# epsilla-cloud/vectordb

Measured on AMD Instinct MI355X. Metric: QPS @ recall@10>=0.999, 10Mx768 L2, higher is better.
Workload: dtype f32 (exact fp32 distances; the batched scan runs an int8 MFMA pass (int32 accumulation) over an 8-bit mirror of the rows as a lower-bound filter, survivors re-ranked in fp32)

## Files before the change

### vectordb_amd/csrc/flat_kernels.hip

```cpp
#include "kernels.hpp"
#include "stream8_kernel.hpp"

namespace eps {

template <int NQ, int KPL>
__device__ __forceinline__ void offer(WaveTopK<KPL> (&list)[NQ], u64 (&thr)[NQ], int q, u64 key, bool valid,
                                      const FilterSpec& f, int k, bool unique) {
  u64 m = __ballot(valid && key < thr[q]);
  while (m) {
    const int l = __ffsll((long long)m) - 1;
    m &= m - 1;
    const u64 x = shfl64(key, l);
    if (x < thr[q] && row_visible(f, key_id(x), key_dist(x))) {
      if (unique) list[q].insert_unique(x); else list[q].insert(x);
      const u64 kth = list[q].entry(k - 1);
      thr[q] = kth < thr[q] ? kth : thr[q];
    }
  }
}

template <int NQ, int KPL, bool VEC4, int U>
__global__ __launch_bounds__(256) void flat_scan_kernel(FlatScanArgs a) {
  extern __shared__ __attribute__((aligned(16))) float smem[];
  const int dim = a.dim;
// ... 445 lines not shown
    if (lost_s) atomicAdd(a.overflow, 1u);
    if (a.fuse & 1) {
      if (cnt_raw > (u32)S8R_CAP || cnt_raw > (u32)a.cap) atomicAdd(a.overflow, 1u);
      atomicAdd(a.total, (unsigned long long)cnt);
    }
    a.cand_count[q] = 0;
    if (a.pub) {
      __threadfence();
      if (atomicAdd(a.pub_ticket, 1u) == gridDim.x - 1) {
        const u32 ov = atomicAdd(a.overflow, 0u);
        const unsigned long long tot = atomicAdd(a.total, 0ull);
        a.pub[0] = ov;
        a.pub[2] = (u32)tot;
        a.pub[3] = (u32)(tot >> 32);
        __threadfence_system();
        if (a.s8_reset) {
          *a.overflow = 0u;
          *a.total = 0ull;
          *a.pub_ticket = 0u;
        }
      }
    }
  }
}

void launch_rerank(const RerankArgs& a, hipStream_t s) {
  if (a.nq <= 0) return;
  if (a.s8_G && a.s8_fast && pick_kpl(a.k) == 1 && a.s8_waves <= S8_MAX_WAVES && !a.T_next && !a.gsync) {
    const bool v4 = (a.dim % 4 == 0) && ((reinterpret_cast<uintptr_t>(a.rows) & 15) == 0);
    const size_t sm = (size_t)((a.dim + 3) & ~3) * sizeof(float) + (size_t)S8R_CAP * sizeof(u64);
    if (v4) hipLaunchKernelGGL((s8_rerank_kernel<true>), dim3((unsigned)a.nq), dim3(1024), sm, s, a);
    else hipLaunchKernelGGL((s8_rerank_kernel<false>), dim3((unsigned)a.nq), dim3(1024), sm, s, a);
    return;
  }
  const bool vec4 = (a.dim % 4 == 0) && ((reinterpret_cast<uintptr_t>(a.rows) & 15) == 0);
  const int kpl = pick_kpl(a.k);
  const int nw = (a.nq <= 64 && kpl <= 4) ? 16 : 4;
  const size_t shm = (size_t)((a.dim + 3) & ~3) * sizeof(float) + (size_t)nw * kpl * 64 * sizeof(u64);
#define EPS_CASE(KPL_)                                                                                               \
  if (kpl == KPL_) {                                                                                                 \
    if (nw == 16) {                                                                                                  \
      if (vec4) hipLaunchKernelGGL((rerank_kernel<KPL_, true, 16>), dim3((unsigned)a.nq), dim3(1024), shm, s, a);    \
      else hipLaunchKernelGGL((rerank_kernel<KPL_, false, 16>), dim3((unsigned)a.nq), dim3(1024), shm, s, a);        \
    } else {                                                                                                         \
      if (vec4) hipLaunchKernelGGL((rerank_kernel<KPL_, true, 4>), dim3((unsigned)a.nq), dim3(256), shm, s, a);      \
      else hipLaunchKernelGGL((rerank_kernel<KPL_, false, 4>), dim3((unsigned)a.nq), dim3(256), shm, s, a);          \
    }                                                                                                                \
    return;                                                                                                          \
  }
  EPS_CASE(1) EPS_CASE(2) EPS_CASE(4) EPS_CASE(8) EPS_CASE(16)
#undef EPS_CASE
}

__global__ void finalize_kernel(const u64* run_keys, int64_t nq, int k, int64_t id_base, int64_t id_stride,
                                int64_t* ids, float* dist, int32_t* counts) {
  const int64_t i = (int64_t)blockIdx.x * blockDim.x + threadIdx.x;
  if (i >= nq * k) return;
  const u64 key = run_keys[i];
  const bool valid = key != KEY_EMPTY;
  ids[i] = valid ? (int64_t)key_id(key) * id_stride + id_base : -1;
  dist[i] = valid ? key_dist(key) : __builtin_inff();
  if (counts && (i % k) == 0) {
    int c = 0;
    for (int e = 0; e < k; ++e) c += run_keys[i + e] != KEY_EMPTY;
    counts[i / k] = c;
  }
}
void launch_finalize(const u64* run_keys, int64_t nq, int k, int64_t id_base, int64_t id_stride, int64_t* ids,
                     float* dist, int32_t* counts, hipStream_t s) {
  const int64_t n = nq * k;
  if (n <= 0) return;
  hipLaunchKernelGGL(finalize_kernel, dim3((unsigned)((n + 255) / 256)), dim3(256), 0, s, run_keys, nq, k, id_base,
                     id_stride, ids, dist, counts);
}

__global__ void fill_u64_kernel(u64* p, int64_t n, u64 v) {
  const int64_t i = (int64_t)blockIdx.x * blockDim.x + threadIdx.x;
  if (i < n) p[i] = v;
}
void launch_fill_u64(u64* p, int64_t n, u64 v, hipStream_t s) {
  if (n <= 0) return;
  hipLaunchKernelGGL(fill_u64_kernel, dim3((unsigned)((n + 255) / 256)), dim3(256), 0, s, p, n, v);
}

__global__ __launch_bounds__(256) void normalize_kernel(float* rows, int64_t n, int dim, int only_if_nonzero) {
  const int64_t r = (int64_t)blockIdx.x * 4 + (threadIdx.x >> 6);
  if (r >= n) return;
  const int lane = lane_id();
  float* p = rows + r * dim;
  float s = 0.f;
  for (int c = lane; c < dim; c += 64) s = fmaf(p[c], p[c], s);
  for (int o = 32; o > 0; o >>= 1) s += __shfl_xor(s, o);
  if (only_if_nonzero && !(s > 1e-10f)) return;
  const float nrm = sqrtf(s);
  for (int c = lane; c < dim; c += 64) p[c] = p[c] / nrm;
}
void launch_normalize(float* rows, int64_t n, int dim, bool only_if_nonzero, hipStream_t s) {
  if (n <= 0) return;
  hipLaunchKernelGGL(normalize_kernel, dim3((unsigned)((n + 3) / 4)), dim3(256), 0, s, rows, n, dim,
                     only_if_nonzero ? 1 : 0);
}

__global__ void merge_shards_kernel(const float* dist, const int64_t* ids, int shards, int64_t nq, int k,
                                    float* out_dist, int64_t* out_ids, int64_t stride_bytes, int32_t* out_counts) {
  const int64_t q = (int64_t)blockIdx.x * blockDim.x + threadIdx.x;
  if (q >= nq) return;
// ... 40 lines not shown
```

### vectordb_amd/csrc/kernels.hpp

```cpp
#pragma once
#include <hip/hip_runtime.h>
#include <stdint.h>

#include "device_common.hpp"

namespace eps {

struct FlatScanArgs {
  const float* rows;
  int64_t row_begin, row_end;
  int dim;
  int metric;
  const float* queries;
  int64_t nq;
  int k;
  FilterSpec f;
  u64* partial;
  int W;
  const u64* thr_in;
  const u64* lo_in;
  int64_t lo_stride;
};
int flat_scan_waves(int64_t nrows, int64_t nq, int dim);
void launch_flat_scan(const FlatScanArgs& a, hipStream_t s);

void launch_merge_lists(const u64* keys, int slots, int k, int64_t nq, u64* run_keys, bool merge_run, hipStream_t s,
                        const u32* counts = nullptr, const FilterSpec* visible = nullptr, u64 id_stride = 0, u32 id_head = 0,
                        u32* seed_cand = nullptr, int seed_cap = 0, u32* seed_cnt = nullptr);

struct RerankArgs {
  const float* rows;
  int dim;
  int metric;
  const float* queries;
  int64_t nq;
  int k;
  FilterSpec f;
  const u32* cand;
  u32* cand_count;
  int cap;
  u64* run_keys;
  int fuse;
  u32* overflow;
  unsigned long long* total;
  void* T_next;
  const float* qstat;
  const float* scal;
  int bits;
  float u, slack;
  u32* gsync;
  int64_t* fin_ids = nullptr;
  float* fin_dist = nullptr;
  int32_t* fin_counts = nullptr;
  int64_t fin_base = 0, fin_stride = 1;
  const int* s8_G = nullptr;
  int s8_slots = 64;
  const u32* s8_counts = nullptr;
  const u64* s8_lists = nullptr;
  int s8_waves = 0;
  u32* s8_cand = nullptr;
  u32* pub = nullptr;
  u32* pub_ticket = nullptr;
  int s8_fast = 0;
  int s8_reset = 0;
};
void launch_rerank(const RerankArgs& a, hipStream_t s);

void launch_finalize(const u64* run_keys, int64_t nq, int k, int64_t id_base, int64_t id_stride, int64_t* ids,
                     float* dist, int32_t* counts, hipStream_t s);

void launch_normalize(float* rows, int64_t n, int dim, bool only_if_nonzero, hipStream_t s);
void launch_merge_shards(const float* dist, const int64_t* ids, int shards, int64_t nq, int k, float* out_dist,
                         int64_t* out_ids, hipStream_t s, int64_t stride_bytes = 0, int32_t* out_counts = nullptr);
void launch_fill_u64(u64* p, int64_t n, u64 v, hipStream_t s);

constexpr int SEL_ROWS = 1024;
constexpr int SEL_THREADS = 256;
constexpr int SEL_SCAN_THREADS = 512;
inline int64_t select_blocks(int64_t n) { return (n + SEL_ROWS - 1) / SEL_ROWS; }
struct SelectArgs {
  FilterSpec f;
  int64_t n;
  int64_t skip, limit;
  int64_t id_base, id_stride;
  u64* bits;
  u32* counts;
  int64_t* offsets;
  int64_t* ids_out;
  int64_t* count_out;
  int64_t* total_out;
};
void launch_select(const SelectArgs& a, hipStream_t s);

}
```

### vectordb_amd/csrc/mfma_filter.hip

```cpp
#include <algorithm>
#include <cmath>
#include <cstdio>
#include <cstring>
#include <numeric>
#include <vector>

#include "mirror.hpp"
#include "mfma_kernels.hpp"

namespace eps {

__global__ __launch_bounds__(256) void query_prep_kernel(const float* q, int64_t nq, int64_t b_pad, int dim, int d_pad,
                                                         _Float16* qh, float* qstat) {
  const int64_t r = (int64_t)blockIdx.x * 4 + (threadIdx.x >> 6);
  if (r >= b_pad) return;
  const int lane = lane_id();
  _Float16* dst = qh + r * d_pad;
  if (r >= nq) {
    for (int c = lane; c < d_pad; c += 64) dst[c] = (_Float16)0.f;
    if (lane == 0) qstat[r * 4 + 0] = qstat[r * 4 + 1] = qstat[r * 4 + 2] = qstat[r * 4 + 3] = 0.f;
    return;
  }
  const float* src = q + r * dim;
  float s2 = 0.f, e2 = 0.f;
// ... 116 lines not shown
    if (i8)
      while (nstages < 8 && (double)k * 5.0 * std::pow((double)n / (double)S0, 1.0 / (double)nstages) > 0.5 * (double)cap) ++nstages;
    const double r = std::max(i8 ? 3.0 : 4.0, std::pow((double)n / (double)S0, 1.0 / (double)nstages));
    const int64_t qt = std::max<int64_t>(1, b_pad / 256);
    const int64_t unit = 256 * std::max<int64_t>(1, 256 / std::gcd<int64_t>(256, qt));
    double f = 1.0;
    for (int st = 1; st < nstages; ++st) {
      f *= r;
      int64_t bnd = (int64_t)((double)S0 * f) / ROWPAD * ROWPAD;
      if (bnd >= 2 * unit) bnd = bnd / unit * unit;
      if (bnd < n && bnd > bounds.back()) bounds.push_back(bnd);
    }
  } else {
    bounds.push_back(std::min(S0, n));
    for (int64_t bnd : {S0 * 32, S0 * 256}) {
      if (bnd < n && bnd > bounds.back()) bounds.push_back(bnd);
    }
  }
  if (bounds.back() < n) bounds.push_back(n);
  return bounds;
}

struct Chain {
  const float* dq; int64_t nq; int k; u64* run_keys;
  bool i8;
  bool approx;
  int64_t n;
  bool fold;
  bool seeded;
  bool prologue;
  bool gsync;
  int version;
  int64_t b_pad, S0;
  int cap;
  int d_pad_h;
  float u8, slack;
  CallCounters c;
  FilterSpec fs;
  std::vector<int64_t> bounds;
  bool prep_does_it_all() const { return i8 && version >= 7; }
  const float* maxima(const HalfMirror& m) const { return i8 ? (fold ? m.scal8f.as<float>() : m.scal8.as<float>()) : m.scal.as<float>(); }
  u32* group_counters(const HalfMirror& m) const { return gsync ? m.gsync.as<u32>() : nullptr; }
};

static int32_t plan_chain(Index& ix, HalfMirror& m, const float* dq, int64_t nq, int k, u64* run_keys, bool approx, int cap_scale, bool i8, int64_t n, Chain* out) {
  Chain& c = *out = Chain{dq, nq, k, run_keys, i8, approx, n};
  c.b_pad = (nq + BN3 - 1) / BN3 * BN3;
  c.cap = std::max(4096, 64 * k) * cap_scale;
  c.d_pad_h = i8 ? m.d_pad8 / 2 : m.d_pad;
  c.u8 = key_unit8(ix.metric_, m.step8);
  c.slack = rerank_slack(ix.dim_);
  const int64_t b_pad = c.b_pad;
  if (!m.qstat.reserve((size_t)b_pad * 16) || !m.T.reserve((size_t)b_pad * 4) || !m.cand.reserve((size_t)nq * c.cap * 8) ||
      !m.cnt.reserve((size_t)(nq + 4) * 4 + 16) || !m.seedc.reserve((size_t)nq * k * 4) || !(i8 ? m.q8.reserve((size_t)b_pad * m.d_pad8) : m.qh.reserve((size_t)b_pad * m.d_pad * 2)))
    return ix.fail(EPS_INFRA_UNEXPECTED_ERROR, "MFMA engine: out of device memory (scratch)");
  c.version = (c.d_pad_h % 128 != 0 || c.d_pad_h < 256) ? 3 : 7;
  if (c.version >= 7 && !m.qf.reserve((size_t)b_pad * c.d_pad_h * 2)) return ix.fail(EPS_INFRA_UNEXPECTED_ERROR, "MFMA engine: out of device memory (scratch)");
  if (!m.gsync.reserve(1024)) return ix.fail(EPS_INFRA_UNEXPECTED_ERROR, "MFMA engine: out of device memory (scratch)");
  c.S0 = seed_rows(k);
  c.seeded = !(tune_int("EPS_MFMA_SEED", 1) == 0) && n > 4 * c.S0;
  c.prologue = c.seeded && c.version >= 7;
  c.gsync = !(tune_int("EPS_MFMA_GROUPSYNC", 1) == 0);
  c.fold = i8 && !approx && m.fold8;
  c.c = call_counters(m.cnt.as<u32>(), nq);
  c.fs = ix.filter_spec();
  c.bounds = plan_stages(n, nq, k, b_pad, c.cap, i8, approx, c.seeded);
  return EPS_OK;
}

static int32_t prepare_queries(Index& ix, HalfMirror& m, const Chain& c) {
  hipStream_t s = ix.stream_;
  if (c.i8) {
    Prep8Extra px;
    if (c.prep_does_it_all()) {
      px.qf = m.qf.as<signed char>();
      if (c.prologue) {
        px.T2 = reinterpret_cast<u64*>(m.T.p);
        px.n2 = c.b_pad / 2;
        px.Tv = 0x7F8000007F800000ull;
        px.cnt = c.c.cnt;
        px.cntv = (u32)c.S0;
        px.gsync = c.group_counters(m);
      }
    }
    const hipError_t er = prep8_queries(m, c.fold, (int)ix.dim_, ix.metric_, c.dq, c.nq, c.b_pad, m.q8.as<signed char>(), m.qstat.as<float>(), px, s);
    if (er != hipSuccess) return ix.hip_fail(er, "memset");
    if (c.fold) ix.stats_.i8_folded = 1;
    ix.stats_.i8_rotated = m.rot8 ? 1 : 0;
  } else {
    hipLaunchKernelGGL(query_prep_kernel, dim3((unsigned)((c.b_pad + 3) / 4)), dim3(256), 0, s, c.dq, c.nq, c.b_pad, (int)ix.dim_,
                       m.d_pad, m.qh.as<_Float16>(), m.qstat.as<float>());
  }
  if (c.version >= 7 && !c.prep_does_it_all())
    hipLaunchKernelGGL(pack_qf_kernel, dim3((unsigned)((c.b_pad / 32) * (c.d_pad_h / 16))), dim3(64), 0, s, m.qh.as<_Float16>(), m.qf.as<_Float16>(), c.b_pad, c.d_pad_h);
  return EPS_OK;
}

static FilterArgs filter_args(const Index& ix, const HalfMirror& m, const Chain& c) {
  const bool i8 = c.i8;
  FilterArgs fa;
  fa.xh = i8 ? reinterpret_cast<const _Float16*>(m.x8.p) : m.xh.as<_Float16>();
  fa.qh = i8 ? reinterpret_cast<const _Float16*>(m.q8.p) : m.qh.as<_Float16>();
  fa.qf = m.qf.as<_Float16>();
  fa.base = i8 ? (c.fold ? m.acc0b.as<float>() : m.acc0.as<float>()) : (ix.metric_ == 0 ? m.xn.as<float>() : m.zeros.as<float>());
  fa.base_s = i8 ? (c.fold ? m.acc0b.as<float>() : m.acc0.as<float>()) : (ix.metric_ == 0 ? m.xn_s.as<float>() : m.zeros_s.as<float>());
  fa.T = m.T.as<float>();
  fa.d_pad = c.d_pad_h;
// ... 59 lines not shown
  hipStream_t s = ix.stream_;
  const bool i8 = c.i8;
  const int64_t S0 = c.S0;
  u32* cnt = c.c.cnt;
  const bool dense = c.version >= 7;
  if (c.prologue && c.prep_does_it_all()) {
  } else if (c.prologue) {
    const int64_t cells = std::max<int64_t>(std::max<int64_t>(c.b_pad / 2, c.nq), 256);
    hipLaunchKernelGGL(seed_prologue_kernel, dim3((unsigned)((cells + 255) / 256)), dim3(256), 0, s, reinterpret_cast<u64*>(m.T.p), c.b_pad / 2, 0x7F8000007F800000ull,
                       cnt, c.nq, (u32)S0, c.group_counters(m));
  } else {
    launch_fill_u64(reinterpret_cast<u64*>(m.T.p), c.b_pad / 2, 0x7F8000007F800000ull, s);
    const hipError_t er = dense ? hipMemsetD32Async(reinterpret_cast<hipDeviceptr_t>(cnt), (int)S0, (size_t)c.nq, s) : hipMemsetAsync(cnt, 0, (size_t)c.nq * 4, s);
    if (er != hipSuccess) return ix.hip_fail(er, "memset");
  }
  unsigned long long seed_stride = 0;
  u32 seed_head = 0;
  FilterArgs f0 = fa;
  f0.dense = dense ? 1 : 0;
  f0.cand_keys = m.cand.as<u64>();
  if (!c.approx) {
    const u32 sample_head = (u32)(S0 / 2);
    const unsigned long long sample_stride = (unsigned long long)(((unsigned __int128)(c.n - sample_head) << 32) / (unsigned __int128)(S0 - sample_head));
    int64_t& smp_version = i8 ? m.sample8_version : m.sample_version;
    int64_t& smp_n = i8 ? m.sample8_n : m.sample_n;
    int64_t& smp_rows = i8 ? m.sample8_rows : m.sample_rows;
    DevBuf& smp_x = i8 ? m.sx8 : m.sxh;
    DevBuf& smp_base = i8 ? m.sacc0 : m.sbase;
    DevBuf& smp_base_u = i8 ? m.sacc0 : m.sbase_u;
    if (smp_version != ix.rows_version_ || smp_n != c.n || smp_rows != S0) {
      if (!smp_x.reserve((size_t)S0 * c.d_pad_h * 2) || !smp_base.reserve((size_t)S0 * 4) || !smp_base_u.reserve((size_t)S0 * 4))
        return ix.fail(EPS_INFRA_UNEXPECTED_ERROR, "MFMA engine: out of device memory (seed sample)");
      hipLaunchKernelGGL(seed_sample_kernel, dim3((unsigned)S0), dim3(256), 0, s, fa.xh, i8 ? m.acc0.as<u32>() : reinterpret_cast<const u32*>(fa.base_s),
                         i8 ? m.acc0.as<u32>() : reinterpret_cast<const u32*>(fa.base),
                         sample_stride, sample_head, c.d_pad_h, smp_x.as<_Float16>(), smp_base.as<u32>(), smp_base_u.as<u32>());
      smp_version = ix.rows_version_;
      smp_n = c.n;
      smp_rows = S0;
    }
    f0.xh = smp_x.as<_Float16>();
    f0.base_s = smp_base.as<float>();
    f0.base = smp_base_u.as<float>();
    seed_stride = sample_stride;
    seed_head = sample_head;
  }
  f0.tile0 = 0;
  f0.ntiles = (S0 + BM3 - 1) / BM3;
  f0.row_hi = S0;
  launch_filter(m, c, f0, s);
  if (c.approx) {
    launch_merge_lists(f0.cand_keys, c.cap, c.k, c.nq, c.run_keys, false, s, cnt, nullptr, seed_stride, seed_head);
    return EPS_OK;
  }
  launch_merge_lists(f0.cand_keys, c.cap, c.k, c.nq, c.run_keys, false, s, cnt, &c.fs, seed_stride, seed_head, m.seedc.as<u32>(), c.k, cnt);
  ra.cand = m.seedc.as<u32>();
  ra.cap = c.k;
  ra.fuse = 2;
  ra.T_next = m.T.p;
  launch_rerank(ra, s);
  return EPS_OK;
}

static void dump_stage(const HalfMirror& m, const Chain& c, size_t st, int64_t ntiles, hipStream_t s) {
  const int64_t nq = c.nq;
  const int k = c.k;
  std::vector<u32> hc((size_t)nq);
  std::vector<float> hT((size_t)nq);
  std::vector<u64> hk((size_t)nq * k);
  (void)hipMemcpyAsync(hc.data(), c.c.cnt, (size_t)nq * 4, hipMemcpyDeviceToHost, s);
  (void)hipMemcpyAsync(hT.data(), m.T.p, (size_t)nq * 4, hipMemcpyDeviceToHost, s);
  (void)hipMemcpyAsync(hk.data(), c.run_keys, (size_t)nq * k * 8, hipMemcpyDeviceToHost, s);
  (void)hipStreamSynchronize(s);
  u32 mn = ~0u, mx = 0; double sum = 0; float tmin = 3e38f, tmax = -3e38f; int64_t empt = 0, big = 0;
  for (int64_t j = 0; j < nq; ++j) { mn = std::min(mn, hc[j]); mx = std::max(mx, hc[j]); sum += hc[j]; tmin = std::min(tmin, hT[j]); tmax = std::max(tmax, hT[j]); empt += hk[j * k + k - 1] == KEY_EMPTY; big += hc[j] > (u32)c.cap; }
  fprintf(stderr, "[eps] stage %zu rows [%lld,%lld) tiles %lld: cnt min %u mean %.1f max %u (>cap: %lld), T min %g max %g, empty kth %lld, scal %g %g %g\n", st, (long long)c.bounds[st], (long long)c.bounds[st + 1], (long long)ntiles, mn, sum / nq, mx, (long long)big, tmin, tmax, (long long)empt, m.h_scal[0], m.h_scal[1], m.h_scal[2]);
}

static void run_stage(Index& ix, HalfMirror& m, const Chain& c, size_t st, FilterArgs fa, RerankArgs ra, bool* fin_done) {
  hipStream_t s = ix.stream_;
  const int64_t lo = c.bounds[st], hi = c.bounds[st + 1];
  const bool fused = !c.approx;
  const bool have_T = fused && (st > 0 || c.seeded);
  const int pad_only = have_T ? 1 : 0;
  if ((!have_T || st == 0) && !(have_T && c.i8 && c.prologue)) {
    const dim3 grid((unsigned)((c.b_pad + 255) / 256));
    if (c.i8)
      hipLaunchKernelGGL(threshold8_kernel, grid, dim3(256), 0, s, c.run_keys, c.k, c.nq, c.b_pad, m.qstat.as<float>(), c.maxima(m), ix.metric_, c.u8, m.T.as<int>(), c.c.cnt,
                         m.gsync.as<u32>(), c.slack, c.approx ? 1 : 0, pad_only);
    else
      hipLaunchKernelGGL(threshold_kernel, grid, dim3(256), 0, s, c.run_keys, c.k, c.nq, c.b_pad, m.qstat.as<float>(), c.maxima(m), ix.metric_, m.T.as<float>(), c.c.cnt,
                         m.gsync.as<u32>(), c.slack, c.approx ? 1 : 0, pad_only);
  }
  fa.tile0 = lo / BM3;
  fa.ntiles = (hi + BM3 - 1) / BM3 - fa.tile0;
  fa.row_hi = hi;
  const bool biggest = (st + 2 == c.bounds.size());
  if (biggest) {
    (void)hipEventRecord(ix.evk0_, s);
    ix.stats_.main_kernel_rows = hi - lo;
    ix.stats_.main_kernel_queries = c.nq;
    ix.stats_.main_kernel_bits = c.i8 ? 8 : 16;
  }
  const int sev = (!c.approx && c.nq >= 256 && ix.stage_n_ < Index::STAGE_EV) ? ix.stage_n_++ : -1;
  if (sev >= 0) (void)hipEventRecord(ix.stage_ev_[sev][0], s);
  launch_filter(m, c, fa, s);
  if (sev >= 0) {
    (void)hipEventRecord(ix.stage_ev_[sev][1], s);
    ix.stats_.filter_rows_all += hi - lo;
  }
  if (biggest) (void)hipEventRecord(ix.evk1_, s);
  if (!fused) hipLaunchKernelGGL(stage_counts_kernel, dim3((unsigned)((c.nq + 255) / 256)), dim3(256), 0, s, c.c.cnt, c.nq, c.cap, c.c.overflow, c.c.total);
// ... 299 lines not shown
```

### vectordb_amd/csrc/mfma_kernels.hpp

```cpp
#pragma once
#include <hip/hip_runtime.h>
#include <stdint.h>

#include <type_traits>

#include "device_common.hpp"

namespace eps {

typedef _Float16 half8 __attribute__((ext_vector_type(8)));
typedef float f32x16 __attribute__((ext_vector_type(16)));
typedef int i32x16 __attribute__((ext_vector_type(16)));


struct FilterArgs {
  const _Float16* xh;
  const _Float16* qh;
  const _Float16* qf;
  const float* base;
  const float* base_s;
  int dense;
  u32* group_sync;
  int sync_shift;
  const float* T;
// ... 359 lines not shown
  };
  lane_values();

  const int64_t a_stride = (int64_t)8 * G * TR * ldk;
  int ri_c = 0, qi_c = 0;
  int ri_n = 0, qi_n = 0;
  advance(ri_n, qi_n);
  const _Float16* A_t = rows_of(0);
  const _Float16* A_n = ntile > 1 ? rows_of(ri_n) : A_t;
  const _Float16* B_t = frags_of(0);
  const _Float16* B_n = (nqt > 1 && ntile > 1) ? frags_of(qi_n) : B_t;
  u32* wcnt = reinterpret_cast<u32*>(lds + RING * ASLOT + 2048 + 4096) + wave * 4;
  u64* wbuf = reinterpret_cast<u64*>(lds + RING * ASLOT + 2048 + 4096 + 64) + wave * V7_CAPW;
  float* wkey = reinterpret_cast<float*>(lds + RING * ASLOT + 2048 + 4096 + 64 + 4 * V7_CAPW * 8) + wave * V7_CAPW;
  volatile __attribute__((address_space(3))) u32* wcnt_lds = (volatile __attribute__((address_space(3))) u32*)wcnt;
  if (MODE != FM_DENSE && lane == 0) *wcnt = 0;
  auto append = [&](int64_t qq, u32 row, float dapx) __attribute__((always_inline)) {
    const u32 slot_c = atomicAdd(&a.cnt[qq], 1u);
    if (slot_c < (u32)a.cap) {
      if (MODE == FM_KEYS) a.cand_keys[qq * (int64_t)a.cap + slot_c] = make_key(dapx, row);
      else a.cand[qq * (int64_t)a.cap + slot_c] = row;
    }
  };
  auto flush = [&]() __attribute__((always_inline)) {
    u32 ln;
    asm volatile("v_mbcnt_lo_u32_b32 %0, -1, 0\n\tv_mbcnt_hi_u32_b32 %0, -1, %0" : "=v"(ln));
    u32 n = *wcnt_lds;
    n = n < (u32)V7_CAPW ? n : (u32)V7_CAPW;
    for (u32 e = ln; e < n; e += 64) {
      const u64 v = wbuf[e];
      append((int64_t)(v >> 32), (u32)v, MODE == FM_KEYS ? wkey[e] : 0.f);
    }
    if (ln == 0) *wcnt_lds = 0;
  };
  const bool rendezvous = a.group_sync && a.tiles_q <= per_xcd;
  u32* gs_ctr = a.group_sync + (xcd * G + rg);
  const int64_t sync_mask = ((int64_t)1 << a.sync_shift) - 1;
  if (rendezvous && wave == 0 && lane == 0) __hip_atomic_fetch_add(gs_ctr, 1u, __ATOMIC_RELAXED, __HIP_MEMORY_SCOPE_AGENT);
  asm volatile("s_waitcnt vmcnt(0)" ::: "memory");
  issue_base(0, 0);
#pragma unroll
  for (int it = 0; it < NRB; ++it) issue_piece(A_t, 0, it);
#pragma unroll
  for (int it = 0; it < NRB; ++it) issue_piece(A_t + 64, ASLOT, it);
#pragma unroll
  for (int kk = 0; kk < 4; ++kk) {
    EPS_GLOAD_B128(fb[0][kk][0], lane16, B_t + kk * 512, 0);
    if (JQ == 2) EPS_GLOAD_B128(fb[0][kk][JQ - 1], lane16, B_t + jstride + kk * 512, 0);
  }
#pragma unroll
  for (int it = 0; it < NRB; ++it) issue_piece(A_t + 128, 2 * ASLOT, it);
#pragma unroll
  for (int kk = 0; kk < 4; ++kk) {
    EPS_GLOAD_B128(fb[1][kk][0], lane16, B_t + 2048 + kk * 512, 0);
    if (JQ == 2) EPS_GLOAD_B128(fb[1][kk][JQ - 1], lane16, B_t + jstride + 2048 + kk * 512, 0);
  }
  if (JQ == 2) asm volatile("s_waitcnt vmcnt(16)" ::: "memory");
  else asm volatile("s_waitcnt vmcnt(12)" ::: "memory");
  __builtin_amdgcn_s_barrier();
  asm volatile("" ::: "memory");
  EPS_DS_READ_B128(fa[0][0], faddr[0], 0);
  EPS_DS_READ_B128(fa[0][1], faddr[0], 4096);
  EPS_DS_READ_B128(fa[0][2], faddr[0], 8192);
  EPS_DS_READ_B128(fa[0][3], faddr[0], 12288);
  EPS_DS_READ_B128(fa[0][4], faddr[0], 16384);
  EPS_DS_READ_B128(fa[0][5], faddr[0], 20480);
  EPS_DS_READ_B128(fa[0][6], faddr[0], 24576);
  EPS_DS_READ_B128(fa[0][7], faddr[0], 28672);

  const _Float16* pA_run = A_t + 3 * 64;
  int akt_run = 3;
  const _Float16* pB_run = B_t + 2 * 2048;
  int bkt_run = 2;
  u32 sA_run = 0, sN_run = ASLOT, sD_run = 3 * ASLOT;
  u32 ad_run = faddr[1];
  auto step = [&](auto U, auto FIRST) __attribute__((always_inline)) {
    constexpr int rb = decltype(U)::value % 2;
    constexpr bool first = decltype(FIRST)::value;
    const u32 sA = sA_run, sN = sN_run, sD = sD_run;
    const _Float16* pA = pA_run;
    const _Float16* pB = pB_run;
    const _Float16* pA_nx = pA;
    const _Float16* pB_nx = pB;
    int akt_nx = akt_run, bkt_nx = bkt_run;
#pragma unroll
    for (int kk = 0; kk < 4; ++kk) {
      const int cur = kk & 1, nxt = cur ^ 1;
      const u32 ad = ad_run;
#pragma unroll
      for (int i = 0; i < NRB; ++i) {
        const bool has_frag = (i == 1 || i == 3) && kk > 0 && (i >> 1) < JQ;
        const bool has_dma = i == 5 || i == 7;
        const _Float16* vsrc = nullptr;
        asm volatile("s_waitcnt lgkmcnt(7)" ::: "memory");
        __builtin_amdgcn_sched_barrier(0);
        if (JQ == 2 && first && kk == 0) {
          if (i < VI) V7Asm<I8>::v2(acc[i][JQ - 1], fa[cur][i], fb[rb][kk][JQ - 1], acc[i][0]);
          else V7Asm<I8>::a2(acc[i][JQ - 1], fa[cur][i], fb[rb][kk][JQ - 1], acc[i][0]);
        } else {
          if (i < VI) V7Asm<I8>::v(acc[i][0], fa[cur][i], fb[rb][kk][0]);
          else V7Asm<I8>::a_(acc[i][0], fa[cur][i], fb[rb][kk][0]);
        }
        __builtin_amdgcn_sched_barrier(0);
        {
          switch (i) {
            case 0: EPS_DS_READ_B128(fa[nxt][0], ad, 0); break;
            case 1: EPS_DS_READ_B128(fa[nxt][1], ad, 4096); break;
            case 2: EPS_DS_READ_B128(fa[nxt][2], ad, 8192); break;
            case 3: EPS_DS_READ_B128(fa[nxt][3], ad, 12288); break;
            case 4: EPS_DS_READ_B128(fa[nxt][4], ad, 16384); break;
            case 5: EPS_DS_READ_B128(fa[nxt][5], ad, 20480); break;
            case 6: EPS_DS_READ_B128(fa[nxt][6], ad, 24576); break;
            default: EPS_DS_READ_B128(fa[nxt][7], ad, 28672); break;
          }
        }
        if (has_frag) {
          vsrc = pB + (i >> 1) * jstride + (kk - 1) * 512;
          asm volatile("" : "+s"(vsrc));
        } else if (has_dma) {
          vsrc = prep_piece(pA, sD, kk * 2 + (i >> 1) - 2);
        }
        if (i == NRB - 1) {
          u32 adn = faddr[(kk + 2) & 3] + (kk < 2 ? sA : sN);
          asm volatile("" : "+v"(adn));
          ad_run = adn;
        }
        if (kk == 3 && i == NRB - 2) {
          akt_nx = akt_run + 1;
          pA_nx = pA + 64;
          if (akt_nx == KT) {
            akt_nx = 0;
            pA_nx = A_n;
          }
          bkt_nx = bkt_run + 1;
          pB_nx = pB + 2048;
          if (bkt_nx == KT) {
            bkt_nx = 0;
            pB_nx = B_n;
          }
        }
        __builtin_amdgcn_sched_barrier(0);
        if (JQ == 2) {
          if (first && kk == 0) {
            if (i < VI) V7Asm<I8>::v(acc[i][0], fa[cur][i], fb[rb][kk][0]);
            else V7Asm<I8>::a_(acc[i][0], fa[cur][i], fb[rb][kk][0]);
          } else {
            if (i < VI) V7Asm<I8>::v(acc[i][JQ - 1], fa[cur][i], fb[rb][kk][JQ - 1]);
            else V7Asm<I8>::a_(acc[i][JQ - 1], fa[cur][i], fb[rb][kk][JQ - 1]);
          }
        }
        __builtin_amdgcn_sched_barrier(0);
        if (has_frag) EPS_GLOAD_B128(fb[rb][kk - 1][(i >> 1) % JQ], lane16, vsrc, 0);
        else if (has_dma) fire_piece(vsrc);
      }
    }
    {
      EPS_GLOAD_B128(fb[rb][3][0], lane16, pB + 3 * 512, 0);
      if (JQ == 2) EPS_GLOAD_B128(fb[rb][3][JQ - 1], lane16, pB + jstride + 3 * 512, 0);
    }
    pA_run = pA_nx;
    akt_run = akt_nx;
    pB_run = pB_nx;
    bkt_run = bkt_nx;
    sA_run = sN;
    sN_run = (sN + ASLOT) & (RING * ASLOT - 1);
    sD_run = sA;
    if (JQ == 2) asm volatile("s_waitcnt vmcnt(16)" ::: "memory");
    else asm volatile("s_waitcnt vmcnt(12)" ::: "memory");
    __builtin_amdgcn_s_barrier();
    asm volatile("" ::: "memory");
  };

  for (int64_t t = 0; t < ntile; ++t) {
    const int64_t row0 = (a.tile0 + tile_rt(ri_c)) * TR;
    const int64_t qbase = (int64_t)tile_qt(qi_c) * QT + wave * (32 * JQ);
    lane_values();
    ad_run = faddr[1] + sA_run;
    if (rendezvous && wave == 0 && (t & sync_mask) == 0) {
      const u32 want = (u32)QTB * (u32)((t >> a.sync_shift) + 1);
      for (int spin = 0; spin < 1024; ++spin) {
        u32 seen;
        asm volatile("s_load_dword %0, %1, 0x0 glc\n\ts_waitcnt lgkmcnt(0)" : "=s"(seen) : "s"(gs_ctr) : "memory");
        if (seen >= want) break;
        __builtin_amdgcn_s_sleep(2);
      }
    }
    if (nqt > 1 && t > 0) {
#pragma unroll
      for (int j = 0; j < JQ; ++j) {
        const int64_t qjt = (int64_t)tile_qt(qi_c) * QT + wave * (32 * JQ) + j * 32 + ((lane16 >> 4) & 31);
        tq_lds[j * 64 + (lane16 >> 4)] = I8 ? a.T[qjt] : a.T[qjt] * a.inv_s;
        float cm;
        {
          const int sv = a.metric == 1 ? 0x3f800000 : 0;
          asm volatile("v_mov_b32 %0, %1" : "=v"(cm) : "s"(sv));
        }
        tq_lds[(2 + j) * 64 + (lane16 >> 4)] = MODE != FM_IDS ? (I8 ? a.qstat[qjt * 4 + 3] : (a.metric == 0 ? a.qstat[qjt * 4] : cm)) : 0.f;
      }
    }
    if (t + 1 < ntile) issue_base(ri_n, (int)((t + 1) & 1));
    auto init_block = [&](int i, int par, int kh4) __attribute__((always_inline)) {
      const float* bl0 = base_lds + par * 256;
      const int rbase = i * 32 + kh4;
#pragma unroll
      for (int gq = 0; gq < 4; ++gq) {
        if (I8) {
          const int4 bv = *reinterpret_cast<const int4*>(&bl0[rbase + 8 * gq]);
          acc[i][0][4 * gq + 0] = bv.x;
          acc[i][0][4 * gq + 1] = bv.y;
          acc[i][0][4 * gq + 2] = bv.z;
          acc[i][0][4 * gq + 3] = bv.w;
        } else {
          const float4 bv = *reinterpret_cast<const float4*>(&bl0[rbase + 8 * gq]);
          acc[i][0][4 * gq + 0] = bv.x;
          acc[i][0][4 * gq + 1] = bv.y;
          acc[i][0][4 * gq + 2] = bv.z;
          acc[i][0][4 * gq + 3] = bv.w;
        }
      }
    };
    {
      const int kh4 = (int)(lane16 >> 7) & 4;
#define EPS_INIT_AT_HEAD(I_)                                                                        \
  {                                                                                                 \
    init_block((I_), (int)(t & 1), kh4);                                                            \
    __builtin_amdgcn_sched_barrier(0);  \
  }
      EPS_INIT_AT_HEAD(0) EPS_INIT_AT_HEAD(1) EPS_INIT_AT_HEAD(2) EPS_INIT_AT_HEAD(3)
      EPS_INIT_AT_HEAD(4) EPS_INIT_AT_HEAD(5) EPS_INIT_AT_HEAD(6) EPS_INIT_AT_HEAD(7)
#undef EPS_INIT_AT_HEAD
    }
    step(std::integral_constant<int, 0>{}, std::true_type{});
    step(std::integral_constant<int, 1>{}, std::false_type{});
    for (int kt = 2; kt < KT; kt += 2) {
      step(std::integral_constant<int, 0>{}, std::false_type{});
      step(std::integral_constant<int, 1>{}, std::false_type{});
    }
    asm volatile("s_nop 15\n\ts_nop 7" ::: "memory");
    if (rendezvous && wave == 0 && t + 1 < ntile && ((t + 1) & sync_mask) == 0 && lane16 == 0) __hip_atomic_fetch_add(gs_ctr, 1u, __ATOMIC_RELAXED, __HIP_MEMORY_SCOPE_AGENT);
    A_t = A_n;
    B_t = B_n;
    ri_c = ri_n;
    qi_c = qi_n;
    {
      const int ri_before = ri_n;
      advance(ri_n, qi_n);
      if (t + 2 < ntile) {
        if (ri_n != ri_before) A_n += a_stride;
        if (nqt > 1) B_n = frags_of(qi_n);
      }
    }
    u32 lne;
    asm volatile("v_mbcnt_lo_u32_b32 %0, -1, 0\n\tv_mbcnt_hi_u32_b32 %0, -1, %0" : "=v"(lne));
    const int l31e = (int)(lne & 31), kh4e = (int)(lne >> 5) * 4;
    thr_t Tq[JQ];
    float cj[JQ];
#pragma unroll
    for (int j = 0; j < JQ; ++j) {
      Tq[j] = __builtin_bit_cast(thr_t, tq_lds[j * 64 + lne]);
      cj[j] = MODE == FM_DENSE ? tq_lds[(2 + j) * 64 + lne] : 0.f;
    }
#pragma unroll
    for (int i0 = 0; i0 < NRB; i0 += GROUP) {
      thr_t mxg[GROUP][JQ];
      bool group_hit = true;
      if (MODE != FM_DENSE) {
        bool h = false;
#pragma unroll
        for (int j = 0; j < JQ; ++j) {
          __builtin_amdgcn_sched_barrier(0);
          thr_t gm = mxg[0][j] = OP::max16(acc[i0][j]);
#pragma unroll
          for (int ii = 1; ii < GROUP; ++ii) {
            __builtin_amdgcn_sched_barrier(0);
            mxg[ii][j] = OP::max16(acc[i0 + ii][j]);
            gm = gm > mxg[ii][j] ? gm : mxg[ii][j];
          }
          h |= gm >= Tq[j];
        }
        group_hit = __any(h);
      }
      if (MODE == FM_DENSE || __builtin_expect(group_hit, 0)) {
#pragma unroll
// ... 79 lines not shown
```

Baseline: 147,900.

## Fuse seed-stage merge and rerank into a single per-query seed_finish kernel

Adds a seed_finish_kernel that, per query block, selects the k-th smallest approximate seed key, collects survivors at or below it in shared memory, builds the candidate id list, reranks those rows in fp32, writes the run keys and sets the next-stage threshold. This replaces the separate merge_lists plus rerank launches in the seeded prologue, which removes one launch and the global round trip through the seedc buffer. The seedc reservation moves to the fallback path, which is used when shared memory would exceed 64KB. The rank-based tau selection assumes that per-thread minima spread well. If k-1 minima are not distinct across threads, tau stays empty and every candidate survives, up to the cap, so candidates can be dropped when the cap overflows.

```diff
diff --git a/vectordb_amd/csrc/flat_kernels.hip b/vectordb_amd/csrc/flat_kernels.hip
--- a/vectordb_amd/csrc/flat_kernels.hip
+++ b/vectordb_amd/csrc/flat_kernels.hip
@@ -521,6 +521,178 @@
 #undef EPS_CASE
 }
 
+template <int KPL, bool VEC4>
+__global__ __launch_bounds__(256) void seed_finish_kernel(RerankArgs a, SeedFinishArgs sf, int surv_cap) {
+  extern __shared__ __attribute__((aligned(16))) float smem[];
+  constexpr int NW = 4, NT = 256, KREG = 16, U = 4;
+  __shared__ u32 ids_s[KPL * 64];
+  __shared__ u64 tau_s;
+  __shared__ u32 surv_n, seeds_n;
+  const int dim = a.dim;
+  const int k = a.k;
+  const int qstride = (dim + 3) & ~3;
+  u64* sh = reinterpret_cast<u64*>(smem + qstride);
+  u64* surv = sh + NW * KPL * 64;
+  const int64_t q = blockIdx.x;
+  const int lane = lane_id();
+  const int wave = threadIdx.x >> 6;
+  const u64* src = sf.keys + q * (int64_t)sf.slots;
+  int total = sf.slots < sf.seeds_max ? sf.slots : sf.seeds_max;
+  total = a.cand_count[q] < (u32)total ? (int)a.cand_count[q] : total;
+  u64 kreg[KREG];
+#pragma unroll
+  for (int j = 0; j < KREG; ++j) {
+    const int i = (int)threadIdx.x + j * NT;
+    kreg[j] = i < total ? src[i] : KEY_EMPTY;
+  }
+  for (int i = threadIdx.x; i < qstride; i += NT) smem[i] = i < dim ? a.queries[q * dim + i] : 0.f;
+  if (a.gsync && q == 0) a.gsync[threadIdx.x] = 0;
+  if (threadIdx.x == 0) {
+    tau_s = KEY_EMPTY;
+    surv_n = 0;
+  }
+  auto seen = [&](u64 key) {
+    return key != KEY_EMPTY && row_visible(a.f, sf.id_stride ? seed_row(key_id(key), sf.id_head, sf.id_stride) : key_id(key), key_dist(key));
+  };
+  u64 mn = KEY_EMPTY;
+#pragma unroll
+  for (int j = 0; j < KREG; ++j) {
+    if (!seen(kreg[j])) kreg[j] = KEY_EMPTY;
+    mn = kreg[j] < mn ? kreg[j] : mn;
+  }
+  for (int i = (int)threadIdx.x + KREG * NT; i < total; i += NT) {
+    const u64 key = src[i];
+    if (key < mn && seen(key)) mn = key;
+  }
+  sh[threadIdx.x] = mn;
+  __syncthreads();
+  if (mn != KEY_EMPTY) {
+    int rank = 0;
+    for (int j0 = 0; j0 < NT; j0 += 8) {
+#pragma unroll
+      for (int jj = 0; jj < 8; ++jj) rank += sh[j0 + jj] < mn ? 1 : 0;
+    }
+    if (rank == k - 1) tau_s = mn;
+  }
+  __syncthreads();
+  const u64 tau = tau_s;
+#pragma unroll
+  for (int j = 0; j < KREG; ++j) {
+    if (kreg[j] != KEY_EMPTY && kreg[j] <= tau) {
+      const u32 slot = atomicAdd(&surv_n, 1u);
+      if (slot < (u32)surv_cap) surv[slot] = kreg[j];
+    }
+  }
+  for (int i = (int)threadIdx.x + KREG * NT; i < total; i += NT) {
+    const u64 key = src[i];
+    if (key <= tau && seen(key)) {
+      const u32 slot = atomicAdd(&surv_n, 1u);
+      if (slot < (u32)surv_cap) surv[slot] = key;
+    }
+  }
+  __syncthreads();
+  const int m = surv_n < (u32)surv_cap ? (int)surv_n : surv_cap;
+  WaveTopK<KPL> L[1];
+  u64 thr[1];
+  L[0].init();
+  thr[0] = KEY_EMPTY;
+  const FilterSpec nof = no_filter();
+  const int rounded = (m + NT - 1) / NT * NT;
+  for (int i = threadIdx.x; i < rounded; i += NT) {
+    const u64 key = i < m ? surv[i] : KEY_EMPTY;
+    offer<1, KPL>(L, thr, 0, key, key != KEY_EMPTY, nof, k, false);
+  }
+  L[0].store(sh + wave * (KPL * 64), k);
+  __syncthreads();
+  if (wave == 0) {
+    for (int w = 1; w < NW; ++w) {
+      for (int e0 = 0; e0 < k; e0 += 64) {
+        const int e = e0 + lane;
+        const u64 key = e < k ? sh[w * (KPL * 64) + e] : KEY_EMPTY;
+        offer<1, KPL>(L, thr, 0, key, key != KEY_EMPTY, nof, k, false);
+      }
+    }
+    int c = 0;
+#pragma unroll
+    for (int r = 0; r < KPL; ++r) {
+      const int e = r * 64 + lane;
+      const u64 key = L[0].key[r];
+      const bool ok = e < k && key != KEY_EMPTY;
+      const unsigned long long mk = __ballot(ok);
+      if (ok) ids_s[c + __popcll(mk & ((1ull << lane) - 1ull))] = sf.id_stride ? seed_row(key_id(key), sf.id_head, sf.id_stride) : key_id(key);
+      c += __popcll(mk);
+    }
+    if (lane == 0) seeds_n = (u32)c;
+  }
+  __syncthreads();
+  const u32 cnt = seeds_n;
+  const int G = group_lanes(dim, VEC4);
+  const int RPW = 64 / G;
+  const int g = lane / G;
+  const int t = lane & (G - 1);
+  L[0].init();
+  thr[0] = KEY_EMPTY;
+  for (u32 c0 = wave * RPW * U; c0 < cnt; c0 += NW * RPW * U) {
+    const float* rp[U];
+    u32 id[U];
+    bool ok[U];
+#pragma unroll
+    for (int u = 0; u < U; ++u) {
+      const u32 ci = c0 + u * RPW + g;
+      ok[u] = ci < cnt;
+      id[u] = ids_s[ok[u] ? ci : cnt - 1];
+      rp[u] = a.rows + (int64_t)id[u] * dim;
+    }
+    float acc[U][1];
+    row_dists<U, 1, VEC4>(rp, smem, qstride, dim, a.metric, G, acc);
+#pragma unroll
+    for (int u = 0; u < U; ++u) {
+      const u64 key = make_key(finish_dist(a.metric, acc[u][0]), id[u]);
+      offer<1, KPL>(L, thr, 0, key, ok[u] && t == 0, a.f, k, true);
+    }
+  }
+  L[0].store(sh + wave * (KPL * 64), k);
+  __syncthreads();
+  if (wave != 0) return;
+  for (int w = 1; w < NW; ++w) {
+    for (int e0 = 0; e0 < k; e0 += 64) {
+      const int e = e0 + lane;
+      const u64 key = e < k ? sh[w * (KPL * 64) + e] : KEY_EMPTY;
+      offer<1, KPL>(L, thr, 0, key, key != KEY_EMPTY, nof, k, true);
+    }
+  }
+  L[0].store(a.run_keys + q * k, k);
+  const u64 kth = L[0].entry(k - 1);
+  if (lane == 0) {
+    a.cand_count[q] = 0;
+    const float* qs = a.qstat + q * 4;
+    if (a.bits == 8) {
+      static_cast<int*>(a.T_next)[q] = kth == KEY_EMPTY ? -(1 << 30) : stage_threshold8(key_dist(kth), qs, a.scal, a.metric, a.u, a.slack, 0);
+    } else {
+      static_cast<float*>(a.T_next)[q] = kth == KEY_EMPTY ? 3.0e38f : stage_threshold16(key_dist(kth), qs, a.scal, a.metric, a.slack, 0);
+    }
+  }
+}
+
+bool launch_seed_finish(const RerankArgs& a, const SeedFinishArgs& sf, hipStream_t s) {
+  if (a.nq <= 0) return true;
+  const int kpl = pick_kpl(a.k);
+  const int64_t per_thread = (sf.seeds_max + 255) / 256;
+  const int64_t surv_cap = std::min<int64_t>((int64_t)a.k * per_thread, sf.seeds_max);
+  const size_t shm = (size_t)((a.dim + 3) & ~3) * sizeof(float) + ((size_t)4 * kpl * 64 + (size_t)surv_cap) * sizeof(u64);
+  if (!a.T_next || surv_cap < 1 || shm + (size_t)kpl * 64 * sizeof(u32) + 64 > 65536) return false;
+  const bool vec4 = (a.dim % 4 == 0) && ((reinterpret_cast<uintptr_t>(a.rows) & 15) == 0);
+#define EPS_CASE(KPL_)                                                                                                                   \
+  if (kpl == KPL_) {                                                                                                                     \
+    if (vec4) hipLaunchKernelGGL((seed_finish_kernel<KPL_, true>), dim3((unsigned)a.nq), dim3(256), shm, s, a, sf, (int)surv_cap);       \
+    else hipLaunchKernelGGL((seed_finish_kernel<KPL_, false>), dim3((unsigned)a.nq), dim3(256), shm, s, a, sf, (int)surv_cap);           \
+    return true;                                                                                                                         \
+  }
+  EPS_CASE(1) EPS_CASE(2) EPS_CASE(4) EPS_CASE(8) EPS_CASE(16)
+#undef EPS_CASE
+  return false;
+}
+
 __global__ void finalize_kernel(const u64* run_keys, int64_t nq, int k, int64_t id_base, int64_t id_stride,
                                 int64_t* ids, float* dist, int32_t* counts) {
   const int64_t i = (int64_t)blockIdx.x * blockDim.x + threadIdx.x;
diff --git a/vectordb_amd/csrc/kernels.hpp b/vectordb_amd/csrc/kernels.hpp
--- a/vectordb_amd/csrc/kernels.hpp
+++ b/vectordb_amd/csrc/kernels.hpp
@@ -66,6 +66,15 @@
 };
 void launch_rerank(const RerankArgs& a, hipStream_t s);
 
+struct SeedFinishArgs {
+  const u64* keys;
+  int slots;
+  int seeds_max;
+  u64 id_stride;
+  u32 id_head;
+};
+bool launch_seed_finish(const RerankArgs& a, const SeedFinishArgs& sf, hipStream_t s);
+
 void launch_finalize(const u64* run_keys, int64_t nq, int k, int64_t id_base, int64_t id_stride, int64_t* ids,
                      float* dist, int32_t* counts, hipStream_t s);
 
diff --git a/vectordb_amd/csrc/mfma_filter.hip b/vectordb_amd/csrc/mfma_filter.hip
--- a/vectordb_amd/csrc/mfma_filter.hip
+++ b/vectordb_amd/csrc/mfma_filter.hip
@@ -192,7 +192,7 @@
   c.slack = rerank_slack(ix.dim_);
   const int64_t b_pad = c.b_pad;
   if (!m.qstat.reserve((size_t)b_pad * 16) || !m.T.reserve((size_t)b_pad * 4) || !m.cand.reserve((size_t)nq * c.cap * 8) ||
-      !m.cnt.reserve((size_t)(nq + 4) * 4 + 16) || !m.seedc.reserve((size_t)nq * k * 4) || !(i8 ? m.q8.reserve((size_t)b_pad * m.d_pad8) : m.qh.reserve((size_t)b_pad * m.d_pad * 2)))
+      !m.cnt.reserve((size_t)(nq + 4) * 4 + 16) || !(i8 ? m.q8.reserve((size_t)b_pad * m.d_pad8) : m.qh.reserve((size_t)b_pad * m.d_pad * 2)))
     return ix.fail(EPS_INFRA_UNEXPECTED_ERROR, "MFMA engine: out of device memory (scratch)");
   c.version = (c.d_pad_h % 128 != 0 || c.d_pad_h < 256) ? 3 : 7;
   if (c.version >= 7 && !m.qf.reserve((size_t)b_pad * c.d_pad_h * 2)) return ix.fail(EPS_INFRA_UNEXPECTED_ERROR, "MFMA engine: out of device memory (scratch)");
@@ -358,11 +358,13 @@
     launch_merge_lists(f0.cand_keys, c.cap, c.k, c.nq, c.run_keys, false, s, cnt, nullptr, seed_stride, seed_head);
     return EPS_OK;
   }
+  ra.fuse = 2;
+  ra.T_next = m.T.p;
+  if (launch_seed_finish(ra, SeedFinishArgs{f0.cand_keys, c.cap, (int)S0, seed_stride, seed_head}, s)) return EPS_OK;
+  if (!m.seedc.reserve((size_t)c.nq * c.k * 4)) return ix.fail(EPS_INFRA_UNEXPECTED_ERROR, "MFMA engine: out of device memory (scratch)");
   launch_merge_lists(f0.cand_keys, c.cap, c.k, c.nq, c.run_keys, false, s, cnt, &c.fs, seed_stride, seed_head, m.seedc.as<u32>(), c.k, cnt);
   ra.cand = m.seedc.as<u32>();
   ra.cap = c.k;
-  ra.fuse = 2;
-  ra.T_next = m.T.p;
   launch_rerank(ra, s);
   return EPS_OK;
 }
```

After: 148,000 (median of 5 runs). Within noise of the previous version (+0.1%).

## Defer last B fragment load into next step and stage accumulator init via LDS reads

Applied to the files above, without the earlier changes.

The kk=3 B-fragment global load is no longer issued as a tail burst after each step. It is now issued in the next step's kk=0 slot, aimed at the other buffer parity, so vmcnt thresholds drop accordingly. Accumulator initialization from the base LDS block is rewritten to stage 128-bit ds_reads into spare fa registers with software pipelining, then move them into acc registers with accvgpr read/mov inline asm. The intent is to remove stalls at step boundaries and tile heads, at the cost of fragile hand-tuned wait counts and LDS address assumptions.

```diff
diff --git a/vectordb_amd/csrc/mfma_kernels.hpp b/vectordb_amd/csrc/mfma_kernels.hpp
--- a/vectordb_amd/csrc/mfma_kernels.hpp
+++ b/vectordb_amd/csrc/mfma_kernels.hpp
@@ -435,11 +435,12 @@
   for (int it = 0; it < NRB; ++it) issue_piece(A_t + 128, 2 * ASLOT, it);
 #pragma unroll
   for (int kk = 0; kk < 4; ++kk) {
+    if (kk == 3) break;
     EPS_GLOAD_B128(fb[1][kk][0], lane16, B_t + 2048 + kk * 512, 0);
     if (JQ == 2) EPS_GLOAD_B128(fb[1][kk][JQ - 1], lane16, B_t + jstride + 2048 + kk * 512, 0);
   }
-  if (JQ == 2) asm volatile("s_waitcnt vmcnt(16)" ::: "memory");
-  else asm volatile("s_waitcnt vmcnt(12)" ::: "memory");
+  if (JQ == 2) asm volatile("s_waitcnt vmcnt(14)" ::: "memory");
+  else asm volatile("s_waitcnt vmcnt(11)" ::: "memory");
   __builtin_amdgcn_s_barrier();
   asm volatile("" ::: "memory");
   EPS_DS_READ_B128(fa[0][0], faddr[0], 0);
@@ -455,6 +456,7 @@
   int akt_run = 3;
   const _Float16* pB_run = B_t + 2 * 2048;
   int bkt_run = 2;
+  const _Float16* pBp_run = B_t + 2048;
   u32 sA_run = 0, sN_run = ASLOT, sD_run = 3 * ASLOT;
   u32 ad_run = faddr[1];
   auto step = [&](auto U, auto FIRST) __attribute__((always_inline)) {
@@ -463,6 +465,7 @@
     const u32 sA = sA_run, sN = sN_run, sD = sD_run;
     const _Float16* pA = pA_run;
     const _Float16* pB = pB_run;
+    const _Float16* pBp = pBp_run;
     const _Float16* pA_nx = pA;
     const _Float16* pB_nx = pB;
     int akt_nx = akt_run, bkt_nx = bkt_run;
@@ -472,7 +475,7 @@
       const u32 ad = ad_run;
 #pragma unroll
       for (int i = 0; i < NRB; ++i) {
-        const bool has_frag = (i == 1 || i == 3) && kk > 0 && (i >> 1) < JQ;
+        const bool has_frag = (i == 1 || i == 3) && (i >> 1) < JQ;
         const bool has_dma = i == 5 || i == 7;
         const _Float16* vsrc = nullptr;
         asm volatile("s_waitcnt lgkmcnt(7)" ::: "memory");
@@ -498,7 +501,7 @@
           }
         }
         if (has_frag) {
-          vsrc = pB + (i >> 1) * jstride + (kk - 1) * 512;
+          vsrc = (kk == 0 ? pBp + 3 * 512 : pB + (kk - 1) * 512) + (i >> 1) * jstride;
           asm volatile("" : "+s"(vsrc));
         } else if (has_dma) {
           vsrc = prep_piece(pA, sD, kk * 2 + (i >> 1) - 2);
@@ -533,14 +536,12 @@
           }
         }
         __builtin_amdgcn_sched_barrier(0);
-        if (has_frag) EPS_GLOAD_B128(fb[rb][kk - 1][(i >> 1) % JQ], lane16, vsrc, 0);
+        if (has_frag && kk == 0) EPS_GLOAD_B128(fb[rb ^ 1][3][(i >> 1) % JQ], lane16, vsrc, 0);
+        else if (has_frag) EPS_GLOAD_B128(fb[rb][(kk + 3) & 3][(i >> 1) % JQ], lane16, vsrc, 0);
         else if (has_dma) fire_piece(vsrc);
       }
     }
-    {
-      EPS_GLOAD_B128(fb[rb][3][0], lane16, pB + 3 * 512, 0);
-      if (JQ == 2) EPS_GLOAD_B128(fb[rb][3][JQ - 1], lane16, pB + jstride + 3 * 512, 0);
-    }
+    pBp_run = pB;
     pA_run = pA_nx;
     akt_run = akt_nx;
     pB_run = pB_nx;
@@ -548,8 +549,8 @@
     sA_run = sN;
     sN_run = (sN + ASLOT) & (RING * ASLOT - 1);
     sD_run = sA;
-    if (JQ == 2) asm volatile("s_waitcnt vmcnt(16)" ::: "memory");
-    else asm volatile("s_waitcnt vmcnt(12)" ::: "memory");
+    if (JQ == 2) asm volatile("s_waitcnt vmcnt(14)" ::: "memory");
+    else asm volatile("s_waitcnt vmcnt(11)" ::: "memory");
     __builtin_amdgcn_s_barrier();
     asm volatile("" ::: "memory");
   };
@@ -582,36 +583,50 @@
       }
     }
     if (t + 1 < ntile) issue_base(ri_n, (int)((t + 1) & 1));
-    auto init_block = [&](int i, int par, int kh4) __attribute__((always_inline)) {
-      const float* bl0 = base_lds + par * 256;
-      const int rbase = i * 32 + kh4;
-#pragma unroll
-      for (int gq = 0; gq < 4; ++gq) {
-        if (I8) {
-          const int4 bv = *reinterpret_cast<const int4*>(&bl0[rbase + 8 * gq]);
-          acc[i][0][4 * gq + 0] = bv.x;
-          acc[i][0][4 * gq + 1] = bv.y;
-          acc[i][0][4 * gq + 2] = bv.z;
-          acc[i][0][4 * gq + 3] = bv.w;
-        } else {
-          const float4 bv = *reinterpret_cast<const float4*>(&bl0[rbase + 8 * gq]);
-          acc[i][0][4 * gq + 0] = bv.x;
-          acc[i][0][4 * gq + 1] = bv.y;
-          acc[i][0][4 * gq + 2] = bv.z;
-          acc[i][0][4 * gq + 3] = bv.w;
-        }
-      }
-    };
     {
-      const int kh4 = (int)(lane16 >> 7) & 4;
-#define EPS_INIT_AT_HEAD(I_)                                                                        \
-  {                                                                                                 \
-    init_block((I_), (int)(t & 1), kh4);                                                            \
-    __builtin_amdgcn_sched_barrier(0);  \
+      u32 bad = lds_base + RING * ASLOT + (u32)(t & 1) * 1024u + ((lane16 >> 5) & 16u);
+      asm volatile("" : "+v"(bad));
+#define EPS_STAGE_BLOCK(S_, I_)                                          \
+  EPS_DS_READ_B128(fa[1][4 * (S_) + 0], bad, (I_) * 128 + 0);            \
+  EPS_DS_READ_B128(fa[1][4 * (S_) + 1], bad, (I_) * 128 + 32);           \
+  EPS_DS_READ_B128(fa[1][4 * (S_) + 2], bad, (I_) * 128 + 64);           \
+  EPS_DS_READ_B128(fa[1][4 * (S_) + 3], bad, (I_) * 128 + 96);
+#define EPS_MOVE_QUAD(S_, I_, GQ_, PRE_)                                                                                   \
+  {                                                                                                                        \
+    const i32x4 sv_ = __builtin_bit_cast(i32x4, fa[1][4 * (S_) + (GQ_)]);                                                  \
+    thr_t t0_, t1_, t2_, t3_;                                                                                              \
+    if ((I_) < VI)                                                                                                         \
+      asm volatile(PRE_ "v_accvgpr_read_b32 %0, %4\n\tv_accvgpr_read_b32 %1, %5\n\tv_accvgpr_read_b32 %2, %6\n\tv_accvgpr_read_b32 %3, %7" \
+                   : "=v"(t0_), "=v"(t1_), "=v"(t2_), "=v"(t3_) : "a"(sv_[0]), "a"(sv_[1]), "a"(sv_[2]), "a"(sv_[3]));    \
+    else {  \
+                                     \
+      asm volatile(PRE_ "v_accvgpr_mov_b32 %0, %1" : "=a"(t0_) : "a"(sv_[0]));                                             \
+      asm volatile("v_accvgpr_mov_b32 %0, %1" : "=a"(t1_) : "a"(sv_[1]));                                                  \
+      asm volatile("v_accvgpr_mov_b32 %0, %1" : "=a"(t2_) : "a"(sv_[2]));                                                  \
+      asm volatile("v_accvgpr_mov_b32 %0, %1" : "=a"(t3_) : "a"(sv_[3]));                                                  \
+    }                                                                                                                      \
+    acc[I_][0][4 * (GQ_) + 0] = t0_;                                                                                       \
+    acc[I_][0][4 * (GQ_) + 1] = t1_;                                                                                       \
+    acc[I_][0][4 * (GQ_) + 2] = t2_;                                                                                       \
+    acc[I_][0][4 * (GQ_) + 3] = t3_;                                                                                       \
   }
-      EPS_INIT_AT_HEAD(0) EPS_INIT_AT_HEAD(1) EPS_INIT_AT_HEAD(2) EPS_INIT_AT_HEAD(3)
-      EPS_INIT_AT_HEAD(4) EPS_INIT_AT_HEAD(5) EPS_INIT_AT_HEAD(6) EPS_INIT_AT_HEAD(7)
-#undef EPS_INIT_AT_HEAD
+#define EPS_MOVE_BLOCK(S_, I_, WAIT_)                           \
+  EPS_MOVE_QUAD(S_, I_, 0, "s_waitcnt lgkmcnt(" #WAIT_ ")\n\t") \
+  EPS_MOVE_QUAD(S_, I_, 1, "") EPS_MOVE_QUAD(S_, I_, 2, "") EPS_MOVE_QUAD(S_, I_, 3, "") __builtin_amdgcn_sched_barrier(0);
+      __builtin_amdgcn_sched_barrier(0);
+      EPS_STAGE_BLOCK(0, 0) EPS_STAGE_BLOCK(1, 1)
+      EPS_MOVE_BLOCK(0, 0, 4) EPS_STAGE_BLOCK(0, 2)
+      EPS_MOVE_BLOCK(1, 1, 4) EPS_STAGE_BLOCK(1, 3)
+      EPS_MOVE_BLOCK(0, 2, 4) EPS_STAGE_BLOCK(0, 4)
+      EPS_MOVE_BLOCK(1, 3, 4) EPS_STAGE_BLOCK(1, 5)
+      EPS_MOVE_BLOCK(0, 4, 4) EPS_STAGE_BLOCK(0, 6)
+      EPS_MOVE_BLOCK(1, 5, 4) EPS_STAGE_BLOCK(1, 7)
+      EPS_MOVE_BLOCK(0, 6, 4)
+      EPS_MOVE_BLOCK(1, 7, 0)
+      asm volatile("s_nop 1" ::: "memory");
+#undef EPS_MOVE_BLOCK
+#undef EPS_MOVE_QUAD
+#undef EPS_STAGE_BLOCK
     }
     step(std::integral_constant<int, 0>{}, std::true_type{});
     step(std::integral_constant<int, 1>{}, std::false_type{});
```

Measured after the change: 147,000 before, 144,700 after. 0.985x the previous value.
